# ToddThomson/Mila

Hardware: AMD Instinct MI355X
Metric: Gemma-4 12B decode tok/s (B=1, context 2048), 1xMI355X (higher is better)
Workload: dtype bf16; 1 GPU; Gemma-4 12B, weight policy bf16, B=1, prefill T=2048 then decode at positions 2048..; decode_mode=graph, replicas=1, parallelism=replicas only (no collective), bounded_local_kv=0

## Files before the change

### mila_amd/csrc/attention.hip

```cpp
#include "common.h"
#include "rms_common.h"
#include "rope_common.h"
#include "internal.h"
#include "attention_generic.h"
#include "attention_tiles.h"
#include "attention_decode_mfma.h"
#include "attention_decode_plan.h"

namespace mila {

__global__ __launch_bounds__(256) void kv_write_bf16_kernel(uint16_t* __restrict__ Kc, uint16_t* __restrict__ Vc,
                                                            const uint16_t* __restrict__ k,
                                                            const uint16_t* __restrict__ v, int64_t total_vec,
                                                            int chunk, int NKV, int HS, int start_pos, int capacity)
{
    const int hv = HS / 8;
    const int64_t stride = (int64_t)gridDim.x * 256;
    for (int64_t i = (int64_t)blockIdx.x * 256 + threadIdx.x; i < total_vec; i += stride)
    {
        const int e = (int)(i % hv);
        int64_t r = i / hv;
        const int n = (int)(r % NKV);
        r /= NKV;
        const int t = (int)(r % chunk);
        const int b = (int)(r / chunk);
        const int row = (start_pos + t) % capacity;
        const size_t dst = ((((size_t)b * NKV + n) * capacity + row) * hv + e) * 8;
        st16(Kc + dst, ld16(k + i * 8));
        st16(Vc + dst, ld16(v + i * 8));
    }
}

struct AttnParams
{
    uint16_t* Y;
    const uint16_t* Q;
    int64_t q_b_stride;
    uint16_t* K;
    uint16_t* V;
    float* scratch;
    int no_combine;
    const uint8_t* warm_a; int64_t warm_a_lines; int warm_a_blocks;
    const uint8_t* warm_b; int64_t warm_b_lines; int warm_b_blocks; int64_t warm_b_pair;
    uint32_t* tickets;
    int NH, NKV, capacity, position, window, splits;
    float scale;
    const int32_t* pos_dev;
    int flat;
    int64_t raw_b_stride;
    const uint16_t* q_raw;
    const uint16_t* k_raw;
    const uint16_t* v_raw;
    const uint16_t* qw;
    const uint16_t* kw;
    const uint16_t* vw;
    const float* cos_cache;
    const float* sin_cache;
    float eps;
};

template <int EPL>
__device__ __forceinline__ void load_row(uint32_t (&dst)[EPL / 2], const uint16_t* p)
{
    if constexpr (EPL == 8)
    {
        const u32x4 v = ld16(p);
        dst[0] = v[0]; dst[1] = v[1]; dst[2] = v[2]; dst[3] = v[3];
    }
    else if constexpr (EPL == 4)
    {
        const u32x2 v = *reinterpret_cast<const u32x2*>(p);
        dst[0] = v[0]; dst[1] = v[1];
    }
    else
    {
        dst[0] = *reinterpret_cast<const uint32_t*>(p);
    }
}

constexpr int kDecodeWaves = 8;

template <int HS>
__device__ __forceinline__ void head_row_post(const uint16_t* __restrict__ src, const uint16_t* __restrict__ w, bool rotate,
                                              const float* cos_row, const float* sin_row, float eps,
                                              uint16_t* dst_lds, uint16_t* dst_glb)
{
    constexpr int hv = HS / 16;
    const int lane = threadIdx.x & 63;
    const bool act = lane < hv;
    const int l2 = act ? lane : 0;
    const u32x4 xlo = ld16(src + (size_t)l2 * 8), xhi = ld16(src + (size_t)(l2 + hv) * 8);
    u32x4 wlo = u32x4{0u, 0u, 0u, 0u}, whi = wlo;
    if (w) { wlo = ld16(w + (size_t)l2 * 8); whi = ld16(w + (size_t)(l2 + hv) * 8); }
    const float rstd = rms_rstd_wave(src, HS, eps);
    if (act)
    {
        u32x4 lo, hi;
        if (w) { lo = rms_apply8(xlo, wlo, rstd, 0.0f); hi = rms_apply8(xhi, whi, rstd, 0.0f); }
        else { lo = rms_apply8_now(xlo, rstd); hi = rms_apply8_now(xhi, rstd); }
        if (rotate) rope_rotate8_vals(lo, hi, cos_row, sin_row, lane * 8);
        if (dst_lds) { st16(dst_lds + (size_t)lane * 8, lo); st16(dst_lds + (size_t)(lane + hv) * 8, hi); }
        if (dst_glb) { st16(dst_glb + (size_t)lane * 8, lo); st16(dst_glb + (size_t)(lane + hv) * 8, hi); }
    }
}

template <bool SC1>
__device__ __forceinline__ float partial_ld(const float* p)
{
    if constexpr (SC1)
        return __hip_atomic_load((const __attribute__((address_space(1))) float*)p, __ATOMIC_RELAXED, __HIP_MEMORY_SCOPE_AGENT);
    else
        return *p;
}
template <bool SC1>
__device__ __forceinline__ uint16_t combine_dim(const float* __restrict__ base, int HS, int splits, int d)
{
    const int STR = HS + 4;
    const int s = threadIdx.x & 63;
    float vals[16];
#pragma unroll
    for (int u = 0; u < 16; ++u) vals[u] = (u < splits) ? partial_ld<SC1>(base + (size_t)u * STR + d) : 0.0f;
    const float ms = (s < splits) ? partial_ld<SC1>(base + (size_t)s * STR + HS) : -INFINITY;
    const float ls = (s < splits) ? partial_ld<SC1>(base + (size_t)s * STR + HS + 1) : 0.0f;
    float acc = 0.0f;
    const float M = wave_max(ms);
    const float fs = (ms == -INFINITY) ? 0.0f : __expf(ms - M);
    const float L = wave_sum(ls * fs);
    const int n8 = (splits + 7) & ~7;
    for (int i0 = 0; i0 < n8; i0 += 16)
    {
        if (i0 > 0)
        {
#pragma unroll
            for (int u = 0; u < 16; ++u) vals[u] = (i0 + u < splits) ? partial_ld<SC1>(base + (size_t)(i0 + u) * STR + d) : 0.0f;
        }
#pragma unroll
        for (int u = 0; u < 16; ++u)
        {
            const float f = __uint_as_float(__builtin_amdgcn_readlane(__float_as_uint(fs), min(i0 + u, 63)));
            if (i0 + u < n8) acc = fmaf(vals[u], f, acc);
        }
    }
    return f32_to_bf16_bits(L > 0.0f ? acc / L : 0.0f);
}
__device__ __forceinline__ void partial_st_sc1(float* p, float v)
{
    __hip_atomic_store((__attribute__((address_space(1))) float*)p, v, __ATOMIC_RELAXED, __HIP_MEMORY_SCOPE_AGENT);
}

__device__ __forceinline__ void warm_lines(const uint8_t* __restrict__ base, int64_t nlines, int64_t tid, int64_t nthreads, float* never,
                                           int64_t pair = 0)
{
    uint32_t acc = 0;
    int64_t i = tid;
    auto at = [&](int64_t l) { return pair ? base + (l & 1) * pair + (l >> 1) * 128 : base + l * 128; };
    for (; i + 7 * nthreads < nlines; i += 8 * nthreads)
    {
        uint32_t v[8];
#pragma unroll
        for (int u = 0; u < 8; ++u) v[u] = *reinterpret_cast<const uint32_t*>(at(i + u * nthreads));
#pragma unroll
        for (int u = 0; u < 8; ++u) acc ^= v[u];
    }
    for (; i < nlines; i += nthreads) acc ^= *reinterpret_cast<const uint32_t*>(at(i));
    if (acc == 0x12345679u && never != nullptr) never[0] = 1.0f;
}

template <int HS, int GH, bool FUSED>
__global__ __launch_bounds__(kDecodeWaves * 64) void attn_decode_kernel(const AttnParams p)
{
    constexpr int NW = kDecodeWaves;
    constexpr int EPL = (HS >= 128) ? HS / 64 : 2;
    constexpr int NPAIR = EPL / 2;
    constexpr int ACTIVE = HS / EPL;
    constexpr int STR = HS + 2;
    extern __shared__ __attribute__((aligned(16))) unsigned char smem_raw[];
    float* sm = reinterpret_cast<float*>(smem_raw);
    uint16_t* qs = reinterpret_cast<uint16_t*>(smem_raw + (size_t)NW * GH * STR * sizeof(float));

    const int lane = threadIdx.x & 63, wave = threadIdx.x >> 6;
    const bool owner = lane < ACTIVE;
    const int GS = p.NH / p.NKV, hgroups = GS / GH;
    if (!p.flat && (int)blockIdx.x >= p.splits)
    {
        const int64_t wb = ((int64_t)(blockIdx.x - p.splits) * gridDim.y + blockIdx.y) * gridDim.z + blockIdx.z;
        warm_lines(p.warm_a, p.warm_a_lines, wb * (NW * 64) + threadIdx.x, (int64_t)p.warm_a_blocks * gridDim.y * gridDim.z * (NW * 64),
                   p.scratch);
        return;
    }
    const int ngrp = p.NKV * hgroups;
    const int split = p.flat ? (int)blockIdx.x / ngrp : (int)blockIdx.x, grp = p.flat ? (int)blockIdx.x % ngrp : (int)blockIdx.y;
    const int kvh = grp / hgroups, hg = grp % hgroups;
    const int h0 = kvh * GS + hg * GH;
    const int b = blockIdx.z;
    const int pos = p.pos_dev ? *p.pos_dev : p.position;
    const int len = pos + 1;
    const int band_begin = (p.window > 0) ? max(0, len - p.window) : 0;
    const int band = len - band_begin;
    const int chunk = (band + p.splits - 1) / p.splits;
    const int begin = band_begin + split * chunk;
    const int end = min(begin + chunk, len);
    const bool owns_new = FUSED && pos >= begin && pos < end;

    uint16_t* kbase = p.K + ((size_t)b * p.NKV + kvh) * p.capacity * HS;
    uint16_t* vbase = p.V + ((size_t)b * p.NKV + kvh) * p.capacity * HS;

    constexpr int PG = (HS >= 512) ? 4 : 8;
    struct KVG { uint32_t k[PG][NPAIR], v[PG][NPAIR]; };
    auto load_group = [&](KVG& gbuf, int base) {
#pragma unroll
        for (int j = 0; j < PG; ++j)
        {
            const int pp = base + NW * j;
            if (owner && pp < end && !(FUSED && pp == pos))
            {
                const size_t r = (size_t)(pp % p.capacity) * HS + lane * EPL;
                load_row<EPL>(gbuf.k[j], kbase + r);
                load_row<EPL>(gbuf.v[j], vbase + r);
            }
            else
            {
#pragma unroll
                for (int e = 0; e < NPAIR; ++e) { gbuf.k[j][e] = 0u; gbuf.v[j][e] = 0u; }
            }
        }
    };

    int base = begin + wave;
    KVG ga, gb;
    if (base < end) load_group(ga, base);

    uint32_t q[GH][NPAIR];
    if constexpr (FUSED)
    {
        const int half = HS / 2;
        const float* cos_row = p.cos_cache + (size_t)pos * half;
        const float* sin_row = p.sin_cache + (size_t)pos * half;
        const int nrows = GH + (owns_new ? 2 : 0);
        for (int r = wave; r < nrows; r += NW)
        {
            if (r < GH)
                head_row_post<HS>(p.q_raw + (size_t)b * p.raw_b_stride + (size_t)(h0 + r) * HS, p.qw, true, cos_row, sin_row, p.eps, qs + (size_t)r * HS, nullptr);
            else if (r == GH)
                head_row_post<HS>(p.k_raw + (size_t)b * p.raw_b_stride + (size_t)kvh * HS, p.kw, true, cos_row, sin_row, p.eps, qs + (size_t)GH * HS,
                                  (hg == 0) ? kbase + (size_t)(pos % p.capacity) * HS : nullptr);
            else
                head_row_post<HS>(p.v_raw + (size_t)b * p.raw_b_stride + (size_t)kvh * HS, p.vw, false, cos_row, sin_row, p.eps, qs + (size_t)(GH + 1) * HS,
                                  (hg == 0) ? vbase + (size_t)(pos % p.capacity) * HS : nullptr);
        }
        __syncthreads();
#pragma unroll
        for (int g = 0; g < GH; ++g)
        {
            if (owner) load_row<EPL>(q[g], qs + (size_t)g * HS + lane * EPL);
            else
            {
#pragma unroll
                for (int e = 0; e < NPAIR; ++e) q[g][e] = 0u;
            }
        }
    }
    else
    {
#pragma unroll
        for (int g = 0; g < GH; ++g)
        {
            const uint16_t* qp = p.Q + (size_t)b * (p.q_b_stride ? (size_t)p.q_b_stride : (size_t)p.NH * HS) + (size_t)(h0 + g) * HS + lane * EPL;
            if (owner) load_row<EPL>(q[g], qp);
            else
            {
#pragma unroll
                for (int e = 0; e < NPAIR; ++e) q[g][e] = 0u;
            }
        }
    }

    float m[GH], l[GH], o[GH][EPL];
#pragma unroll
    for (int g = 0; g < GH; ++g)
    {
        m[g] = -INFINITY;
        l[g] = 0.0f;
#pragma unroll
        for (int e = 0; e < EPL; ++e) o[g][e] = 0.0f;
    }

    auto patch_new = [&](KVG& gbuf, int base_) {
        if constexpr (FUSED)
        {
            if (owns_new)
            {
#pragma unroll
                for (int j = 0; j < PG; ++j)
                    if (base_ + NW * j == pos && owner)
                    {
                        load_row<EPL>(gbuf.k[j], qs + (size_t)GH * HS + lane * EPL);
                        load_row<EPL>(gbuf.v[j], qs + (size_t)(GH + 1) * HS + lane * EPL);
                    }
            }
        }
    };
    auto compute_group = [&](const KVG& gbuf, int base_) {
        float sc[PG][GH];
#pragma unroll
        for (int j = 0; j < PG; ++j)
#pragma unroll
            for (int g = 0; g < GH; ++g)
            {
                float a = 0.0f;
#pragma unroll
                for (int e = 0; e < NPAIR; ++e) a = dot2_bf16(as_bf16x2(q[g][e]), as_bf16x2(gbuf.k[j][e]), a);
                sc[j][g] = a;
            }
#pragma unroll
        for (int j = 0; j < PG; ++j)
#pragma unroll
            for (int g = 0; g < GH; ++g) sc[j][g] = wave_sum(sc[j][g]);
#pragma unroll
        for (int g = 0; g < GH; ++g)
        {
            float a[PG], mt = -INFINITY;
#pragma unroll
            for (int j = 0; j < PG; ++j)
            {
                a[j] = (base_ + NW * j < end) ? sc[j][g] * p.scale : -INFINITY;
                mt = fmaxf(mt, a[j]);
            }
            const float mn = fmaxf(m[g], mt);
            const float msafe = (mn == -INFINITY) ? 0.0f : mn;
            const float alpha = __expf(m[g] - msafe);
            float ex[PG], rs = 0.0f;
#pragma unroll
            for (int j = 0; j < PG; ++j) { ex[j] = __expf(a[j] - msafe); rs += ex[j]; }
            l[g] = l[g] * alpha + rs;
            m[g] = mn;
#pragma unroll
            for (int e = 0; e < NPAIR; ++e)
            {
                float lo = o[g][2 * e] * alpha, hi = o[g][2 * e + 1] * alpha;
#pragma unroll
                for (int j = 0; j < PG; ++j)
                {
                    lo = fmaf(ex[j], bf16_lo(gbuf.v[j][e]), lo);
                    hi = fmaf(ex[j], bf16_hi(gbuf.v[j][e]), hi);
                }
                o[g][2 * e] = lo;
                o[g][2 * e + 1] = hi;
            }
        }
    };
    for (;;)
    {
        if (base >= end) break;
        int nb = base + NW * PG;
        if (nb < end) load_group(gb, nb);
        patch_new(ga, base);
        compute_group(ga, base);
        base = nb;
        if (base >= end) break;
        nb = base + NW * PG;
        if (nb < end) load_group(ga, nb);
        patch_new(gb, base);
        compute_group(gb, base);
        base = nb;
    }

#pragma unroll
    for (int g = 0; g < GH; ++g)
    {
        float* dst = sm + ((size_t)wave * GH + g) * STR;
        if (owner)
        {
#pragma unroll
            for (int e = 0; e < EPL; ++e) dst[lane * EPL + e] = o[g][e];
        }
        if (lane == 0) { dst[HS] = m[g]; dst[HS + 1] = l[g]; }
    }
    __syncthreads();
    if (wave < GH)
    {
        const int g = wave;
        float M = -INFINITY;
#pragma unroll
        for (int w = 0; w < NW; ++w) M = fmaxf(M, sm[((size_t)w * GH + g) * STR + HS]);
        float L = 0.0f, acc[EPL];
#pragma unroll
        for (int e = 0; e < EPL; ++e) acc[e] = 0.0f;
#pragma unroll
        for (int w = 0; w < NW; ++w)
        {
            const float* src = sm + ((size_t)w * GH + g) * STR;
            const float mw = src[HS];
            const float f = (mw == -INFINITY) ? 0.0f : __expf(mw - M);
            L += src[HS + 1] * f;
            if (owner)
            {
#pragma unroll
                for (int e = 0; e < EPL; ++e) acc[e] += src[lane * EPL + e] * f;
            }
        }
        const int h = h0 + g;
        if (p.splits == 1)
        {
            const float inv = (L > 0.0f) ? 1.0f / L : 0.0f;
            uint16_t* y = p.Y + ((size_t)b * p.NH + h) * HS + lane * EPL;
            if (owner)
            {
#pragma unroll
                for (int e = 0; e < EPL; e += 2)
                    *reinterpret_cast<uint32_t*>(y + e) = pack_bf16x2(acc[e] * inv, acc[e + 1] * inv);
            }
        }
        else if (p.tickets == nullptr)
        {
            float* dst = p.scratch + (((size_t)b * p.NH + h) * p.splits + split) * (HS + 4);
            if (owner)
            {
#pragma unroll
                for (int e = 0; e < EPL; ++e) dst[lane * EPL + e] = acc[e];
            }
            if (lane == 0) { dst[HS] = M; dst[HS + 1] = L; }
        }
        else
        {
            float* dst = p.scratch + (((size_t)b * p.NH + h) * p.splits + split) * (HS + 4);
            if (owner)
            {
#pragma unroll
                for (int e = 0; e < EPL; ++e) partial_st_sc1(dst + lane * EPL + e, acc[e]);
            }
            if (lane == 0) { partial_st_sc1(dst + HS, M); partial_st_sc1(dst + HS + 1, L); }
            asm volatile("s_waitcnt vmcnt(0)" ::: "memory");
        }
    }
    if (p.splits > 1 && p.tickets != nullptr)
    {
        __shared__ int s_last;
        __syncthreads();
        uint32_t* tk = p.tickets + (size_t)b * gridDim.y + blockIdx.y;
        if (threadIdx.x == 0)
        {
            const uint32_t t = __hip_atomic_fetch_add(tk, 1u, __ATOMIC_ACQ_REL, __HIP_MEMORY_SCOPE_AGENT);
            const int last = (t == (uint32_t)(p.splits - 1));
            if (last) __hip_atomic_store(tk, 0u, __ATOMIC_RELAXED, __HIP_MEMORY_SCOPE_AGENT);
            s_last = last;
        }
        __syncthreads();
        if (s_last)
        {
            for (int idx = threadIdx.x; idx < GH * HS; idx += NW * 64)
            {
                const int g = idx / HS, d = idx % HS;
                const int h = h0 + g;
                const float* base = p.scratch + ((size_t)b * p.NH + h) * p.splits * (HS + 4);
                p.Y[((size_t)b * p.NH + h) * HS + d] = combine_dim<true>(base, HS, p.splits, d);
            }
        }
    }
}

__global__ __launch_bounds__(64) void attn_combine_kernel(uint16_t* __restrict__ Y, const float* __restrict__ scratch, int NH,
                                                          int HS, int splits, const uint8_t* __restrict__ warm, int64_t warm_lines_n, int64_t warm_pair, int flat_gh)
{
    int h = blockIdx.x, zc = blockIdx.z;
    const int b = blockIdx.y;
    if (flat_gh > 0)
    {
        const int ngroups = NH / flat_gh, grp = (int)blockIdx.x % ngroups, r = (int)blockIdx.x / ngroups;
        h = grp * flat_gh + r % flat_gh;
        zc = r / flat_gh;
    }
    else if ((int)blockIdx.z >= HS / 64)
    {
        const int64_t wb = ((int64_t)(blockIdx.z - HS / 64) * gridDim.y + blockIdx.y) * gridDim.x + blockIdx.x;
        warm_lines(warm, warm_lines_n, wb * 64 + threadIdx.x, (int64_t)(gridDim.z - HS / 64) * gridDim.y * gridDim.x * 64, nullptr, warm_pair);
        return;
    }
    const int d = zc * 64 + threadIdx.x;
    const float* base = scratch + ((size_t)b * NH + h) * splits * (HS + 4);
    Y[((size_t)b * NH + h) * HS + d] = combine_dim<false>(base, HS, splits, d);
}


template <int HS>
__global__ __launch_bounds__(256) void attn_decode_mfma_kernel(const AttnParams p)
{
    extern __shared__ __attribute__((aligned(16))) unsigned char smem_mfma[];
    const int pos = p.pos_dev ? *p.pos_dev : p.position;
    const MfmaDecodeArgs a{p.Q, p.q_b_stride, p.scratch, p.NH, p.NKV, p.capacity, pos + 1, p.window, p.splits, p.scale};
    attn_decode_mfma_body<HS>(a, MfmaStageBf16<HS>{p.K, p.V}, smem_mfma);
}

__global__ __launch_bounds__(256) void attn_combine_many_kernel(uint16_t* __restrict__ Y, const float* __restrict__ scratch, int NH, int HS, int splits)
{
    __shared__ float s_acc[4][64], s_m[4], s_l[4];
    const int h = blockIdx.x, b = blockIdx.y, lane = threadIdx.x & 63, wave = threadIdx.x >> 6;
    const int d = blockIdx.z * 64 + lane;
    const int STR = HS + 4;
    const int s0 = wave * 64, n = min(64, splits - s0);
    const float* base = scratch + (((size_t)b * NH + h) * splits + s0) * STR;
    float acc = 0.0f, M = -INFINITY, L = 0.0f;
    if (n > 0)
    {
        float vals[16];
#pragma unroll
        for (int u = 0; u < 16; ++u) vals[u] = (u < n) ? base[(size_t)u * STR + d] : 0.0f;
        const float ms = (lane < n) ? base[(size_t)lane * STR + HS] : -INFINITY;
        const float ls = (lane < n) ? base[(size_t)lane * STR + HS + 1] : 0.0f;
        M = wave_max(ms);
        const float fs = (ms == -INFINITY) ? 0.0f : __expf(ms - M);
        L = wave_sum(ls * fs);
        const int n16 = (n + 15) & ~15;
        for (int i0 = 0; i0 < n16; i0 += 16)
        {
            if (i0 > 0)
            {
#pragma unroll
                for (int u = 0; u < 16; ++u) vals[u] = (i0 + u < n) ? base[(size_t)(i0 + u) * STR + d] : 0.0f;
            }
#pragma unroll
            for (int u = 0; u < 16; ++u)
            {
                const float f = __uint_as_float(__builtin_amdgcn_readlane(__float_as_uint(fs), min(i0 + u, 63)));
                acc = fmaf(vals[u], f, acc);
            }
        }
    }
    s_acc[wave][lane] = acc;
    if (lane == 0) { s_m[wave] = M; s_l[wave] = L; }
    __syncthreads();
    if (wave == 0)
    {
        float Mt = fmaxf(fmaxf(s_m[0], s_m[1]), fmaxf(s_m[2], s_m[3]));
        float Lt = 0.0f, out = 0.0f;
#pragma unroll
        for (int w = 0; w < 4; ++w)
        {
            const float f = (s_m[w] == -INFINITY) ? 0.0f : __expf(s_m[w] - Mt);
            Lt = fmaf(s_l[w], f, Lt);
            out = fmaf(s_acc[w][lane], f, out);
        }
        Y[((size_t)b * NH + h) * HS + d] = f32_to_bf16_bits(Lt > 0.0f ? out / Lt : 0.0f);
    }
}

enum DecodeForm { DF_SCALAR, DF_MFMA, DF_GENERIC };
struct DecodePlan
{
    DecodeForm form;
    int splits, band_max;
    int gh, hgroups;
    int flat;
    bool prologue;
    size_t partial_floats;
    size_t scratch_need;
};

constexpr int kMaxSplits = 64;
constexpr int kMaxSplitsMfma = 256;
static int g_tune_positions_per_split = 64;
MILA_TUNE("attn.positions_per_split", g_tune_positions_per_split);
static int g_attn_max_wgs = 256;
MILA_TUNE("attn.max_workgroups", g_attn_max_wgs);
static int g_attn_gh512 = 2;
MILA_TUNE("attn.heads_per_group_512", g_attn_gh512);
static int g_tune_decode_mfma = 1;
MILA_TUNE("attn.mfma_decode", g_tune_decode_mfma);
static int g_tune_kvfp8_mfma = 1;
MILA_TUNE("attn.kvfp8_mfma_decode", g_tune_kvfp8_mfma);
static int g_mfma_min_band = 8192;
MILA_TUNE("attn.mfma_min_band", g_mfma_min_band);
static int g_attn_xcd_local = 0;
MILA_TUNE("attn.xcd_local", g_attn_xcd_local);

static int band_bucket(int len, int capacity)
{
    int b = 4096;
    while (b < len && b < capacity) b <<= 1;
    return min(b, capacity);
}
static int heads_per_group(int GS, int HS) { return HS >= 512 ? (GS >= g_attn_gh512 && g_attn_gh512 == 4 ? 4 : (GS >= 2 ? 2 : 1)) : (GS >= 4 ? 4 : GS); }
static int decode_splits(int B, int NKV, int hgroups, int band)
{
    const int cap = max(1, g_attn_max_wgs / (NKV * hgroups * B));
    const int pps = g_tune_positions_per_split >= 8 ? g_tune_positions_per_split : 64;
    return max(1, min(min((band + pps - 1) / pps, cap), kMaxSplits));
}
static bool mfma_decode_applies(int NH, int NKV, int HS, int band_max)
{
    return g_tune_decode_mfma && HS == 512 && NKV > 0 && (NH / NKV) % 16 == 0 && band_max >= g_mfma_min_band;
}
static int mfma_decode_splits(int B, int NH, int NKV, int band_max)
{
    const int groups = NKV * ((NH / NKV) / 16) * B;
    const int s = (band_max + 127) / 128;
    return max(1, min(min(s, max(1, kNumCU / groups)), kMaxSplitsMfma));
}
static size_t decode_scratch_bytes(int B, int NH, int HS, int splits, bool q_rows)
{
    return (size_t)B * NH * splits * (HS + 4) * sizeof(float) + (q_rows ? (size_t)B * NH * HS * 2 : 0);
}

static DecodePlan plan_decode(int B, int NH, int NKV, int HS, int capacity, int window, int len_hint, bool fused, bool hooks, bool kvfp8 = false)
{
    const bool scalar_only = kvfp8 && !g_tune_kvfp8_mfma;
    DecodePlan d{};
    const int GS = NH / NKV;
    const bool split_kernel = HS == 64 || HS == 128 || HS == 256 || HS == 512;
    d.band_max = (window > 0 && window < capacity) ? window : (len_hint > 0 ? band_bucket(len_hint, capacity) : capacity);
    d.gh = heads_per_group(GS, HS);
    d.hgroups = GS / d.gh;
    if (mfma_decode_applies(NH, NKV, HS, d.band_max) && !hooks && !scalar_only)
    {
        d.form = DF_MFMA;
        d.splits = mfma_decode_splits(B, NH, NKV, d.band_max);
        d.prologue = fused;
    }
    else
    {
        d.form = split_kernel ? DF_SCALAR : DF_GENERIC;
        d.splits = decode_splits(B, NKV, d.hgroups, d.band_max);
        d.flat = (g_attn_xcd_local && split_kernel && (NKV * d.hgroups) % 8 == 0 && !hooks) ? 1 : 0;
    }
    d.partial_floats = (size_t)B * NH * d.splits * (HS + 4);
    d.scratch_need = (d.form == DF_MFMA || (d.form == DF_SCALAR && d.splits > 1)) ? decode_scratch_bytes(B, NH, HS, d.splits, d.prologue) : 0;
    return d;
}
int launch_attn_combine_many(uint16_t* Y, const float* partials, int B, int NH, int HS, int splits, hipStream_t s)
{
    hipLaunchKernelGGL(attn_combine_many_kernel, dim3(NH, B, HS / 64), dim3(256), 0, s, Y, partials, NH, HS, splits);
    return check_hip(hipGetLastError(), "attn_combine_many");
}
static int launch_decode_mfma(const AttnParams& p, int B, hipStream_t s)
{
    constexpr int HS = 512;
    note_form("attn_decode_mfma");
    static bool attr_set = false;
    const size_t lds = mfma_decode_lds_bytes<HS>();
    if (!attr_set)
    {
        int rc = check_hip(hipFuncSetAttribute(reinterpret_cast<const void*>(attn_decode_mfma_kernel<HS>), hipFuncAttributeMaxDynamicSharedMemorySize, (int)lds), "hipFuncSetAttribute(attn_decode_mfma)");
        if (rc) return rc;
        attr_set = true;
    }
    const int n16 = (p.NH / p.NKV) / 16;
    hipLaunchKernelGGL((attn_decode_mfma_kernel<HS>), dim3(p.splits, p.NKV * n16, B), dim3(256), lds, s, p);
    int rc = check_hip(hipGetLastError(), "attn_decode_mfma");
    if (rc) return rc;
    return launch_attn_combine_many(p.Y, p.scratch, B, p.NH, HS, p.splits, s);
}

template <int HS, int GH, bool FUSED>
static int launch_decode(const AttnParams& p, int B, hipStream_t s)
{
    const int hgroups = (p.NH / p.NKV) / GH;
    note_form("attn_decode");
    const size_t lds = (size_t)kDecodeWaves * GH * (HS + 2) * sizeof(float) + (size_t)(GH + 2) * HS * 2;
    const int wa = (p.warm_a && p.warm_a_lines > 0) ? p.warm_a_blocks : 0;
    if (p.flat)
    {
        hipLaunchKernelGGL((attn_decode_kernel<HS, GH, FUSED>), dim3(p.NKV * hgroups * p.splits, 1, B), dim3(kDecodeWaves * 64), lds, s, p);
        int rc = check_hip(hipGetLastError(), "attn_decode (xcd-local)");
        if (rc || p.splits <= 1) return rc;
        hipLaunchKernelGGL(attn_combine_kernel, dim3(p.NH * (HS / 64), B, 1), dim3(64), 0, s, p.Y, p.scratch, p.NH, HS, p.splits, nullptr, 0, 0, GH);
        return check_hip(hipGetLastError(), "attn_combine (xcd-local)");
    }
    hipLaunchKernelGGL((attn_decode_kernel<HS, GH, FUSED>), dim3(p.splits + wa, p.NKV * hgroups, B), dim3(kDecodeWaves * 64), lds, s, p);
    int rc = check_hip(hipGetLastError(), "attn_decode");
    if (rc) return rc;
    if (p.splits > 1 && !p.no_combine && !p.tickets)
    {
        const int wbk = (p.warm_b && p.warm_b_lines > 0) ? p.warm_b_blocks : 0;
        hipLaunchKernelGGL(attn_combine_kernel, dim3(p.NH, B, HS / 64 + wbk), dim3(64), 0, s, p.Y, p.scratch, p.NH, HS, p.splits, p.warm_b,
                           p.warm_b_lines, p.warm_b_pair, 0);
        rc = check_hip(hipGetLastError(), "attn_combine");
    }
    return rc;
}

template <int HS, bool FUSED>
static int dispatch_gs(const AttnParams& p, int B, hipStream_t s)
{
    const int GS = p.NH / p.NKV;
    if (GS != 1 && GS != 2 && GS != 4 && GS != 8 && GS != 16 && GS != 32)
        return set_error(MILA_E_UNSUPPORTED, "attention: group size %d (NH/NKV) must be 1,2,4,8,16 or 32", GS);
    switch (heads_per_group(GS, HS))
    {
        case 1: return launch_decode<HS, 1, FUSED>(p, B, s);
        case 2: return launch_decode<HS, 2, FUSED>(p, B, s);
        default: return launch_decode<HS, 4, FUSED>(p, B, s);
    }
}

template <bool FUSED>
static int dispatch_hs(int HS, const AttnParams& p, int B, hipStream_t s)
{
    switch (HS)
    {
        case 64: return dispatch_gs<64, FUSED>(p, B, s);
        case 128: return dispatch_gs<128, FUSED>(p, B, s);
        case 256: return dispatch_gs<256, FUSED>(p, B, s);
        case 512: return dispatch_gs<512, FUSED>(p, B, s);
        default:
            if constexpr (!FUSED)
            {
                if (p.pos_dev) return set_error(MILA_E_UNSUPPORTED, "attention: the device-position form needs a head size of 64, 128, 256 or 512 (got %d)", HS);
                const int64_t qbs = p.q_b_stride ? p.q_b_stride : (int64_t)p.NH * HS;
                GenericAttnParams g{p.Y, p.Q, p.K, p.V, qbs, qbs, (int64_t)p.NKV * p.capacity * HS, (int64_t)p.capacity * HS, HS,
                                    B, 1, p.NH, p.NKV, HS, p.capacity, p.position, p.window, p.scale};
                return launch_attn_generic(g, s);
            }
            return set_error(MILA_E_UNSUPPORTED, "attention: head size %d must be 64, 128, 256 or 512", HS);
    }
}

static int run_decode(const DecodePlan& d, AttnParams p, int B, int HS, size_t scratch_bytes, const char* who, hipStream_t stream)
{
    const bool fused = p.q_raw != nullptr;
    p.splits = d.splits;
    p.flat = d.flat;
    if (d.scratch_need && (!p.scratch || scratch_bytes < d.scratch_need))
        return set_error(MILA_E_SCRATCH_TOO_SMALL, "%s: scratch %zu bytes < required %zu", who, scratch_bytes, d.scratch_need);
    if (d.form != DF_MFMA) return fused ? dispatch_hs<true>(HS, p, B, stream) : dispatch_hs<false>(HS, p, B, stream);
    if (d.prologue)
    {
        uint16_t* q_tmp = reinterpret_cast<uint16_t*>(p.scratch + d.partial_floats);
        for (int b = 0; b < B; ++b)
        {
            uint16_t* kc = p.K + (size_t)b * p.NKV * p.capacity * HS;
            uint16_t* vc = p.V + (size_t)b * p.NKV * p.capacity * HS;
            const size_t ro = (size_t)b * p.raw_b_stride;
            const int rc = p.pos_dev ? mila_cdna4_fused_qkv_post_devpos(q_tmp + (size_t)b * p.NH * HS, kc, vc, p.q_raw + ro, p.k_raw + ro, p.v_raw + ro, p.qw, p.kw, p.vw, p.cos_cache,
                                                                        p.sin_cache, p.NH, p.NKV, HS, p.pos_dev, p.capacity, p.eps, reinterpret_cast<mila_stream_t>(stream))
                                     : mila_cdna4_fused_qkv_post(q_tmp + (size_t)b * p.NH * HS, kc, vc, p.q_raw + ro, p.k_raw + ro, p.v_raw + ro, p.qw, p.kw, p.vw, p.cos_cache,
                                                                 p.sin_cache, p.NH, p.NKV, HS, p.position, p.capacity, p.eps, reinterpret_cast<mila_stream_t>(stream));
            if (rc) return rc;
        }
        p.Q = q_tmp;
        p.q_b_stride = 0;
    }
    return launch_decode_mfma(p, B, stream);
}

static int unfused_decode(const char* who, uint16_t* Y, const uint16_t* Q, int64_t q_b_stride, const uint16_t* Kc, const uint16_t* Vc, void* scratch, size_t scratch_bytes, int B,
                          int NH, int NKV, int HS, int capacity, int position, const int32_t* pos_dev, int len_hint, int window, float scale, hipStream_t stream)
{
    AttnParams p{};
    p.Y = Y; p.Q = Q; p.q_b_stride = q_b_stride; p.K = const_cast<uint16_t*>(Kc); p.V = const_cast<uint16_t*>(Vc); p.scratch = reinterpret_cast<float*>(scratch);
    p.NH = NH; p.NKV = NKV; p.capacity = capacity; p.position = position; p.pos_dev = pos_dev; p.window = window; p.scale = scale;
    return run_decode(plan_decode(B, NH, NKV, HS, capacity, window, len_hint, false, false), p, B, HS, scratch_bytes, who, stream);
}

enum { FD_BATCH = 1, FD_TICKETS = 2, FD_PARTIALS = 4 };
static int fused_decode(const char* who, const mila_fused_attn_args& a, int B, int64_t raw_b_stride, int flags, hipStream_t stream)
{
    MILA_REQUIRE((a.Y || (flags & FD_PARTIALS)) && a.Kc && a.Vc && a.q_raw && a.k_raw && a.v_raw && a.qw && a.kw && a.cos_cache && a.sin_cache &&
                 (a.tickets || !(flags & FD_TICKETS)), "%s: null pointer", who);
    if (flags & FD_BATCH)
    {
        MILA_REQUIRE(B > 0 && a.NH > 0 && a.NKV > 0 && a.NH % a.NKV == 0, "%s: bad sizes (B=%d NH=%d NKV=%d)", who, B, a.NH, a.NKV);
        MILA_REQUIRE(B == 1 || raw_b_stride >= (int64_t)a.NKV * a.HS, "%s: raw_b_stride %lld is shorter than a K row", who, (long long)raw_b_stride);
    }
    else
        MILA_REQUIRE(a.NH > 0 && a.NKV > 0 && a.NH % a.NKV == 0, "%s: bad head counts (NH=%d NKV=%d)", who, a.NH, a.NKV);
    MILA_REQUIRE(a.capacity > 0 && a.window >= 0 && (a.position_dev || a.position >= 0), "%s: bad sizes", who);
    MILA_REQUIRE(a.HS % 16 == 0, "%s: HS=%d must be a multiple of 16", who, a.HS);
    MILA_REQUIRE(a.warm_a_blocks >= 0 && a.warm_a_blocks <= 64 && a.warm_b_blocks >= 0 && a.warm_b_blocks <= 64, "%s: warm block counts must be in [0, 64]", who);
    if (a.tickets)
        MILA_REQUIRE(a.ticket_count >= mila_cdna4_attn_decode_ticket_count(1, a.NH), "%s: %zu tickets < required %zu", who, a.ticket_count,
                     mila_cdna4_attn_decode_ticket_count(1, a.NH));
    AttnParams p{};
    p.Y = a.Y; p.K = a.Kc; p.V = a.Vc; p.scratch = reinterpret_cast<float*>(a.scratch);
    p.NH = a.NH; p.NKV = a.NKV; p.capacity = a.capacity; p.position = a.position; p.pos_dev = a.position_dev; p.window = a.window; p.scale = a.scale;
    p.q_raw = a.q_raw; p.k_raw = a.k_raw; p.v_raw = a.v_raw; p.raw_b_stride = raw_b_stride; p.qw = a.qw; p.kw = a.kw; p.vw = a.vw;
    p.cos_cache = a.cos_cache; p.sin_cache = a.sin_cache; p.eps = a.eps;
    p.tickets = a.tickets;
    p.no_combine = (flags & FD_PARTIALS) ? 1 : 0;
    if (a.warm_a && a.warm_a_bytes >= 128 && a.warm_a_blocks > 0) { p.warm_a = (const uint8_t*)a.warm_a; p.warm_a_lines = (int64_t)(a.warm_a_bytes / 128); p.warm_a_blocks = a.warm_a_blocks; }
    if (a.warm_b && a.warm_b_bytes >= 128 && a.warm_b_blocks > 0) { p.warm_b = (const uint8_t*)a.warm_b; p.warm_b_lines = (int64_t)(a.warm_b_bytes / 128); p.warm_b_blocks = a.warm_b_blocks; p.warm_b_pair = (int64_t)a.warm_b_pair_offset; }
    const DecodePlan d = plan_decode(B, a.NH, a.NKV, a.HS, a.capacity, a.window, a.position_dev ? a.position : a.position + 1, true,
                                     p.tickets || p.no_combine || p.warm_a || p.warm_b);
    if (flags & FD_PARTIALS) MILA_REQUIRE(d.splits > 1, "%s: this (window, capacity) runs unsplit; use fused_attn_decode_bf16", who);
    if (!a.position_dev)
    {
        const int len = a.position + 1, band = (a.window > 0 && a.window < len) ? a.window : len;
        MILA_REQUIRE(band <= a.capacity, "%s: live band %d exceeds the cache capacity %d", who, band, a.capacity);
    }
    return run_decode(d, p, B, a.HS, a.scratch_bytes, who, stream);
}
static mila_fused_attn_args fused_args(uint16_t* Y, uint16_t* Kc, uint16_t* Vc, const uint16_t* q_raw, const uint16_t* k_raw, const uint16_t* v_raw, const uint16_t* qw,
                                       const uint16_t* kw, const uint16_t* vw, const float* cos_cache, const float* sin_cache, void* scratch, size_t scratch_bytes,
                                       uint32_t* tickets, size_t ticket_count, int NH, int NKV, int HS, int capacity, int position, const int32_t* position_dev, int window,
                                       float scale, float eps)
{
    return mila_fused_attn_args{Y, Kc, Vc, q_raw, k_raw, v_raw, qw, kw, vw, cos_cache, sin_cache, scratch, scratch_bytes, tickets, ticket_count, nullptr, 0, 0, nullptr, 0, 0, 0,
                                NH, NKV, HS, capacity, position, position_dev, window, scale, eps};
}

KvFp8DecodeShape plan_decode_kvfp8(int B, int NH, int NKV, int HS, int capacity, int window, int len_hint)
{
    const DecodePlan d = plan_decode(B, NH, NKV, HS, capacity, window, len_hint, false, false, true);
    return KvFp8DecodeShape{d.form == DF_MFMA, d.splits, d.gh, d.hgroups, d.scratch_need};
}
int launch_attn_combine(uint16_t* Y, const float* partials, int B, int NH, int HS, int splits, hipStream_t s)
{
    hipLaunchKernelGGL(attn_combine_kernel, dim3(NH, B, HS / 64), dim3(64), 0, s, Y, partials, NH, HS, splits, nullptr, 0, 0, 0);
    return check_hip(hipGetLastError(), "attn_combine");
}
// ... 206 lines not shown
```

### mila_amd/csrc/rms_common.h

```cpp
#pragma once
#include "common.h"

namespace mila {

__device__ __forceinline__ float sumsq8(const u32x4 v, float acc)
{
#pragma unroll
    for (int d = 0; d < 4; ++d)
    {
        const float lo = bf16_lo(v[d]), hi = bf16_hi(v[d]);
        acc = fmaf(lo, lo, acc);
        acc = fmaf(hi, hi, acc);
    }
    return acc;
}

template <int NW>
__device__ __forceinline__ float rms_rstd_block(const uint16_t* __restrict__ x, int dim, float eps, float* red)
{
    const int lane = threadIdx.x & 63, wib = threadIdx.x >> 6;
    const int nx16 = dim / 8, G = (nx16 + 63) / 64;
    for (int g = wib; g < G; g += NW)
    {
        const int c = 64 * g + lane;
        float s = c < nx16 ? sumsq8(ld16(x + (size_t)c * 8), 0.0f) : 0.0f;
        s = wave_sum(s);
        if (lane == 0) red[g] = s;
    }
    __syncthreads();
    float t = 0.0f;
    for (int g = 0; g < G; ++g) t += red[g];
    return rsqrtf(t / (float)dim + eps);
}
__device__ __forceinline__ float rms_rstd_wave(const uint16_t* __restrict__ x, int dim, float eps)
{
    const int lane = threadIdx.x & 63;
    float ss = 0.0f;
    for (int i = lane; i < dim / 8; i += 64) ss = sumsq8(ld16(x + (size_t)i * 8), ss);
    ss = wave_sum(ss);
    return rsqrtf(ss / (float)dim + eps);
}

__device__ __forceinline__ float rms_apply1(float x, float w, float rstd, float w_offset, float b)
{
    return x * rstd * (w + w_offset) + b;
}
__device__ __forceinline__ u32x4 rms_apply8(const u32x4 x, const u32x4 w, float rstd, float w_offset)
{
    u32x4 y;
#pragma unroll
    for (int d = 0; d < 4; ++d)
        y[d] = pack_bf16x2(rms_apply1(bf16_lo(x[d]), bf16_lo(w[d]), rstd, w_offset, 0.0f),
                           rms_apply1(bf16_hi(x[d]), bf16_hi(w[d]), rstd, w_offset, 0.0f));
    return y;
}
__device__ __forceinline__ u32x4 rms_apply8_bias(const u32x4 x, const u32x4 w, const u32x4 b, float rstd, float w_offset)
{
    u32x4 y;
#pragma unroll
    for (int d = 0; d < 4; ++d)
        y[d] = pack_bf16x2(rms_apply1(bf16_lo(x[d]), bf16_lo(w[d]), rstd, w_offset, bf16_lo(b[d])),
                           rms_apply1(bf16_hi(x[d]), bf16_hi(w[d]), rstd, w_offset, bf16_hi(b[d])));
    return y;
}
__device__ __forceinline__ u32x4 sandwich_tail8(const u32x4 a, const u32x4 rr, float post_scale)
{
    u32x4 r;
#pragma unroll
    for (int d = 0; d < 4; ++d)
    {
        float lo = round_bf16(bf16_lo(rr[d]) + bf16_lo(a[d]));
        float hi = round_bf16(bf16_hi(rr[d]) + bf16_hi(a[d]));
        if (post_scale != 1.0f) { lo = lo * post_scale; hi = hi * post_scale; }
        r[d] = pack_bf16x2(lo, hi);
    }
    return r;
}

__device__ __forceinline__ u32x4 rms_apply8_now(const u32x4 x, float rstd)
{
    u32x4 y;
#pragma unroll
    for (int d = 0; d < 4; ++d)
        y[d] = pack_bf16x2(rms_apply1(bf16_lo(x[d]), 1.0f, rstd, 0.0f, 0.0f), rms_apply1(bf16_hi(x[d]), 1.0f, rstd, 0.0f, 0.0f));
    return y;
}

}
```

Measured before the change: 221.9 tok/s.

## Restructure decode attention prologue to issue loads early and remove divides

Splits the fused q/k/v RMS-norm plus RoPE head-row preprocessing into a request phase and a finish phase. All global loads (rows, weights, cos/sin, first KV group) are issued before any reduction or sync, so their latencies overlap. KV ring indexing switches from per-row modulo to incremental wrap with precomputed steps, head-group math uses host-precomputed shifts and masks, and loads become unconditional with clamped addresses and masking applied afterwards. This removes serialized load latency and integer divides at the cost of extra register pressure and redundant loads for inactive rows. The head-group shift assumes a power-of-two group count, and rms_rstd_wave_request only covers dim up to 512.

```diff
diff --git a/mila_amd/csrc/attention.hip b/mila_amd/csrc/attention.hip
--- a/mila_amd/csrc/attention.hip
+++ b/mila_amd/csrc/attention.hip
@@ -57,6 +57,7 @@
     const float* cos_cache;
     const float* sin_cache;
     float eps;
+    int gs, hgroups, hg_shift, ngrp, ring_step, ring_gstep;
 };
 
 template <int EPL>
@@ -80,25 +81,33 @@
 
 constexpr int kDecodeWaves = 8;
 
+struct HeadRowReq { u32x4 xlo, xhi, wlo, whi, xs; };
 template <int HS>
-__device__ __forceinline__ void head_row_post(const uint16_t* __restrict__ src, const uint16_t* __restrict__ w, bool rotate,
-                                              const float* cos_row, const float* sin_row, float eps,
-                                              uint16_t* dst_lds, uint16_t* dst_glb)
+__device__ __forceinline__ HeadRowReq head_row_request(const uint16_t* __restrict__ src, const uint16_t* __restrict__ w)
 {
     constexpr int hv = HS / 16;
     const int lane = threadIdx.x & 63;
-    const bool act = lane < hv;
-    const int l2 = act ? lane : 0;
-    const u32x4 xlo = ld16(src + (size_t)l2 * 8), xhi = ld16(src + (size_t)(l2 + hv) * 8);
-    u32x4 wlo = u32x4{0u, 0u, 0u, 0u}, whi = wlo;
-    if (w) { wlo = ld16(w + (size_t)l2 * 8); whi = ld16(w + (size_t)(l2 + hv) * 8); }
-    const float rstd = rms_rstd_wave(src, HS, eps);
-    if (act)
+    const int l2 = lane < hv ? lane : 0;
+    const uint16_t* wp = w ? w : src;
+    HeadRowReq r;
+    r.xs = rms_rstd_wave_request(src, HS);
+    r.xlo = ld16(src + (size_t)l2 * 8); r.xhi = ld16(src + (size_t)(l2 + hv) * 8);
+    r.wlo = ld16(wp + (size_t)l2 * 8); r.whi = ld16(wp + (size_t)(l2 + hv) * 8);
+    return r;
+}
+template <int HS>
+__device__ __forceinline__ void head_row_finish(const HeadRowReq& r, bool has_w, bool rotate, f32x4 c0, f32x4 c1, f32x4 s0, f32x4 s1, float eps,
+                                                uint16_t* dst_lds, uint16_t* dst_glb)
+{
+    constexpr int hv = HS / 16;
+    const int lane = threadIdx.x & 63;
+    const float rstd = rms_rstd_wave_finish(r.xs, HS, eps);
+    if (lane < hv)
     {
         u32x4 lo, hi;
-        if (w) { lo = rms_apply8(xlo, wlo, rstd, 0.0f); hi = rms_apply8(xhi, whi, rstd, 0.0f); }
-        else { lo = rms_apply8_now(xlo, rstd); hi = rms_apply8_now(xhi, rstd); }
-        if (rotate) rope_rotate8_vals(lo, hi, cos_row, sin_row, lane * 8);
+        if (has_w) { lo = rms_apply8(r.xlo, r.wlo, rstd, 0.0f); hi = rms_apply8(r.xhi, r.whi, rstd, 0.0f); }
+        else { lo = rms_apply8_now(r.xlo, rstd); hi = rms_apply8_now(r.xhi, rstd); }
+        if (rotate) rope_rotate8_regs(lo, hi, c0, c1, s0, s1);
         if (dst_lds) { st16(dst_lds + (size_t)lane * 8, lo); st16(dst_lds + (size_t)(lane + hv) * 8, hi); }
         if (dst_glb) { st16(dst_glb + (size_t)lane * 8, lo); st16(dst_glb + (size_t)(lane + hv) * 8, hi); }
     }
@@ -117,11 +126,16 @@
 {
     const int STR = HS + 4;
     const int s = threadIdx.x & 63;
+    const int last = splits - 1;
     float vals[16];
 #pragma unroll
-    for (int u = 0; u < 16; ++u) vals[u] = (u < splits) ? partial_ld<SC1>(base + (size_t)u * STR + d) : 0.0f;
-    const float ms = (s < splits) ? partial_ld<SC1>(base + (size_t)s * STR + HS) : -INFINITY;
-    const float ls = (s < splits) ? partial_ld<SC1>(base + (size_t)s * STR + HS + 1) : 0.0f;
+    for (int u = 0; u < 16; ++u) vals[u] = partial_ld<SC1>(base + (size_t)min(u, last) * STR + d);
+    float ms = partial_ld<SC1>(base + (size_t)min(s, last) * STR + HS);
+    float ls = partial_ld<SC1>(base + (size_t)min(s, last) * STR + HS + 1);
+#pragma unroll
+    for (int u = 0; u < 16; ++u) vals[u] = (u < splits) ? vals[u] : 0.0f;
+    ms = (s < splits) ? ms : -INFINITY;
+    ls = (s < splits) ? ls : 0.0f;
     float acc = 0.0f;
     const float M = wave_max(ms);
     const float fs = (ms == -INFINITY) ? 0.0f : __expf(ms - M);
@@ -132,7 +146,9 @@
         if (i0 > 0)
         {
 #pragma unroll
-            for (int u = 0; u < 16; ++u) vals[u] = (i0 + u < splits) ? partial_ld<SC1>(base + (size_t)(i0 + u) * STR + d) : 0.0f;
+            for (int u = 0; u < 16; ++u) vals[u] = partial_ld<SC1>(base + (size_t)min(i0 + u, last) * STR + d);
+#pragma unroll
+            for (int u = 0; u < 16; ++u) vals[u] = (i0 + u < splits) ? vals[u] : 0.0f;
         }
 #pragma unroll
         for (int u = 0; u < 16; ++u)
@@ -178,9 +194,9 @@
     float* sm = reinterpret_cast<float*>(smem_raw);
     uint16_t* qs = reinterpret_cast<uint16_t*>(smem_raw + (size_t)NW * GH * STR * sizeof(float));
 
-    const int lane = threadIdx.x & 63, wave = threadIdx.x >> 6;
+    const int lane = threadIdx.x & 63, wave = __builtin_amdgcn_readfirstlane(threadIdx.x >> 6);
     const bool owner = lane < ACTIVE;
-    const int GS = p.NH / p.NKV, hgroups = GS / GH;
+    const unsigned lane_off = (unsigned)(owner ? lane : 0) * EPL;
     if (!p.flat && (int)blockIdx.x >= p.splits)
     {
         const int64_t wb = ((int64_t)(blockIdx.x - p.splits) * gridDim.y + blockIdx.y) * gridDim.z + blockIdx.z;
@@ -188,91 +204,116 @@
                    p.scratch);
         return;
     }
-    const int ngrp = p.NKV * hgroups;
-    const int split = p.flat ? (int)blockIdx.x / ngrp : (int)blockIdx.x, grp = p.flat ? (int)blockIdx.x % ngrp : (int)blockIdx.y;
-    const int kvh = grp / hgroups, hg = grp % hgroups;
-    const int h0 = kvh * GS + hg * GH;
+    const int split = p.flat ? (int)blockIdx.x / p.ngrp : (int)blockIdx.x, grp = p.flat ? (int)blockIdx.x % p.ngrp : (int)blockIdx.y;
+    const int kvh = grp >> p.hg_shift, hg = grp & (p.hgroups - 1);
+    const int h0 = kvh * p.gs + hg * GH;
     const int b = blockIdx.z;
     const int pos = p.pos_dev ? *p.pos_dev : p.position;
+
+    uint16_t* kbase = p.K + ((size_t)b * p.NKV + kvh) * p.capacity * HS;
+    uint16_t* vbase = p.V + ((size_t)b * p.NKV + kvh) * p.capacity * HS;
+    asm volatile("" ::"s"(kbase), "s"(vbase));
+
+    uint32_t q[GH][NPAIR];
+    HeadRowReq req;
+    bool has_w = false;
+    const uint16_t *idle_k, *idle_v;
+    if constexpr (FUSED)
+    {
+        const size_t rb = (size_t)b * p.raw_b_stride;
+        idle_k = p.k_raw + rb + (size_t)kvh * HS;
+        idle_v = p.v_raw + rb + (size_t)kvh * HS;
+        if (wave < GH + 2)
+        {
+            const uint16_t* src = (wave < GH) ? p.q_raw + rb + (size_t)(h0 + wave) * HS : (wave == GH ? idle_k : idle_v);
+            const uint16_t* w = (wave < GH) ? p.qw : (wave == GH ? p.kw : p.vw);
+            has_w = w != nullptr;
+            req = head_row_request<HS>(src, w);
+        }
+    }
+    else
+    {
+        const uint16_t* qrow = p.Q + (size_t)b * (p.q_b_stride ? (size_t)p.q_b_stride : (size_t)p.NH * HS) + (size_t)h0 * HS;
+        idle_k = idle_v = qrow;
+#pragma unroll
+        for (int g = 0; g < GH; ++g) load_row<EPL>(q[g], qrow + (size_t)g * HS + lane_off);
+        __builtin_amdgcn_sched_barrier(0);
+    }
+
     const int len = pos + 1;
     const int band_begin = (p.window > 0) ? max(0, len - p.window) : 0;
     const int band = len - band_begin;
-    const int chunk = (band + p.splits - 1) / p.splits;
+    const int chunk = (int)((unsigned)(band + p.splits - 1) / (unsigned)p.splits);
     const int begin = band_begin + split * chunk;
     const int end = min(begin + chunk, len);
     const bool owns_new = FUSED && pos >= begin && pos < end;
-
-    uint16_t* kbase = p.K + ((size_t)b * p.NKV + kvh) * p.capacity * HS;
-    uint16_t* vbase = p.V + ((size_t)b * p.NKV + kvh) * p.capacity * HS;
+    const int endc = FUSED ? min(end, pos) : end;
+
+    f32x4 c0 = f32x4{0.0f, 0.0f, 0.0f, 0.0f}, c1 = c0, s0 = c0, s1 = c0;
+    if constexpr (FUSED)
+    {
+        if (wave <= GH)
+        {
+            constexpr int half = HS / 2;
+            const unsigned co = (unsigned)(lane < HS / 16 ? lane : 0) * 8;
+            const float* cos_row = p.cos_cache + (size_t)pos * half;
+            const float* sin_row = p.sin_cache + (size_t)pos * half;
+            c0 = *reinterpret_cast<const f32x4*>(cos_row + co); c1 = *reinterpret_cast<const f32x4*>(cos_row + co + 4);
+            s0 = *reinterpret_cast<const f32x4*>(sin_row + co); s1 = *reinterpret_cast<const f32x4*>(sin_row + co + 4);
+        }
+    }
 
     constexpr int PG = (HS >= 512) ? 4 : 8;
     struct KVG { uint32_t k[PG][NPAIR], v[PG][NPAIR]; };
-    auto load_group = [&](KVG& gbuf, int base) {
+    auto load_group = [&](KVG& gbuf, int base_, unsigned row_) {
+        const bool any = base_ < endc;
+        const uint16_t* kb = any ? kbase : idle_k;
+        const uint16_t* vb = any ? vbase : idle_v;
+        unsigned r = any ? row_ : 0u;
 #pragma unroll
         for (int j = 0; j < PG; ++j)
         {
-            const int pp = base + NW * j;
-            if (owner && pp < end && !(FUSED && pp == pos))
-            {
-                const size_t r = (size_t)(pp % p.capacity) * HS + lane * EPL;
-                load_row<EPL>(gbuf.k[j], kbase + r);
-                load_row<EPL>(gbuf.v[j], vbase + r);
-            }
-            else
-            {
-#pragma unroll
-                for (int e = 0; e < NPAIR; ++e) { gbuf.k[j][e] = 0u; gbuf.v[j][e] = 0u; }
-            }
+            if (j > 0 && base_ + NW * j < endc)
+            {
+                r += (unsigned)p.ring_step;
+                if (r >= (unsigned)p.capacity) r -= (unsigned)p.capacity;
+            }
+            load_row<EPL>(gbuf.k[j], kb + (size_t)r * HS + lane_off);
+            load_row<EPL>(gbuf.v[j], vb + (size_t)r * HS + lane_off);
+        }
+#pragma unroll
+        for (int j = 0; j < PG; ++j)
+        {
+            const bool keep = owner && base_ + NW * j < endc;
+#pragma unroll
+            for (int e = 0; e < NPAIR; ++e) { gbuf.k[j][e] = keep ? gbuf.k[j][e] : 0u; gbuf.v[j][e] = keep ? gbuf.v[j][e] : 0u; }
         }
     };
 
     int base = begin + wave;
+    unsigned row = (unsigned)base % (unsigned)p.capacity;
     KVG ga, gb;
-    if (base < end) load_group(ga, base);
-
-    uint32_t q[GH][NPAIR];
+    load_group(ga, base, row);
+
     if constexpr (FUSED)
     {
-        const int half = HS / 2;
-        const float* cos_row = p.cos_cache + (size_t)pos * half;
-        const float* sin_row = p.sin_cache + (size_t)pos * half;
         const int nrows = GH + (owns_new ? 2 : 0);
-        for (int r = wave; r < nrows; r += NW)
-        {
-            if (r < GH)
-                head_row_post<HS>(p.q_raw + (size_t)b * p.raw_b_stride + (size_t)(h0 + r) * HS, p.qw, true, cos_row, sin_row, p.eps, qs + (size_t)r * HS, nullptr);
-            else if (r == GH)
-                head_row_post<HS>(p.k_raw + (size_t)b * p.raw_b_stride + (size_t)kvh * HS, p.kw, true, cos_row, sin_row, p.eps, qs + (size_t)GH * HS,
-                                  (hg == 0) ? kbase + (size_t)(pos % p.capacity) * HS : nullptr);
-            else
-                head_row_post<HS>(p.v_raw + (size_t)b * p.raw_b_stride + (size_t)kvh * HS, p.vw, false, cos_row, sin_row, p.eps, qs + (size_t)(GH + 1) * HS,
-                                  (hg == 0) ? vbase + (size_t)(pos % p.capacity) * HS : nullptr);
+        if (wave < nrows)
+        {
+            uint16_t* glb = nullptr;
+            if (wave >= GH && hg == 0) glb = (wave == GH ? kbase : vbase) + (size_t)(pos % p.capacity) * HS;
+            head_row_finish<HS>(req, has_w, wave <= GH, c0, c1, s0, s1, p.eps, qs + (size_t)wave * HS, glb);
         }
         __syncthreads();
 #pragma unroll
+        for (int g = 0; g < GH; ++g) load_row<EPL>(q[g], qs + (size_t)g * HS + lane_off);
+    }
+    if (!owner)
+    {
+#pragma unroll
         for (int g = 0; g < GH; ++g)
-        {
-            if (owner) load_row<EPL>(q[g], qs + (size_t)g * HS + lane * EPL);
-            else
-            {
-#pragma unroll
-                for (int e = 0; e < NPAIR; ++e) q[g][e] = 0u;
-            }
-        }
-    }
-    else
-    {
-#pragma unroll
-        for (int g = 0; g < GH; ++g)
-        {
-            const uint16_t* qp = p.Q + (size_t)b * (p.q_b_stride ? (size_t)p.q_b_stride : (size_t)p.NH * HS) + (size_t)(h0 + g) * HS + lane * EPL;
-            if (owner) load_row<EPL>(q[g], qp);
-            else
-            {
-#pragma unroll
-                for (int e = 0; e < NPAIR; ++e) q[g][e] = 0u;
-            }
-        }
+#pragma unroll
+            for (int e = 0; e < NPAIR; ++e) q[g][e] = 0u;
     }
 
     float m[GH], l[GH], o[GH][EPL];
@@ -349,17 +390,23 @@
             }
         }
     };
+    auto next_row = [&](unsigned r) {
+        r += (unsigned)p.ring_gstep;
+        return r >= (unsigned)p.capacity ? r - (unsigned)p.capacity : r;
+    };
     for (;;)
     {
         if (base >= end) break;
         int nb = base + NW * PG;
-        if (nb < end) load_group(gb, nb);
+        row = next_row(row);
+        if (nb < end) load_group(gb, nb, row);
         patch_new(ga, base);
         compute_group(ga, base);
         base = nb;
         if (base >= end) break;
         nb = base + NW * PG;
-        if (nb < end) load_group(ga, nb);
+        row = next_row(row);
+        if (nb < end) load_group(ga, nb, row);
         patch_new(gb, base);
         compute_group(gb, base);
         base = nb;
@@ -651,9 +698,13 @@
 }
 
 template <int HS, int GH, bool FUSED>
-static int launch_decode(const AttnParams& p, int B, hipStream_t s)
-{
+static int launch_decode(const AttnParams& p_in, int B, hipStream_t s)
+{
+    AttnParams p = p_in;
     const int hgroups = (p.NH / p.NKV) / GH;
+    p.gs = p.NH / p.NKV; p.hgroups = hgroups; p.hg_shift = __builtin_ctz((unsigned)hgroups); p.ngrp = p.NKV * hgroups;
+    p.ring_step = kDecodeWaves % p.capacity;
+    p.ring_gstep = (kDecodeWaves * (HS >= 512 ? 4 : 8)) % p.capacity;
     note_form("attn_decode");
     const size_t lds = (size_t)kDecodeWaves * GH * (HS + 2) * sizeof(float) + (size_t)(GH + 2) * HS * 2;
     const int wa = (p.warm_a && p.warm_a_lines > 0) ? p.warm_a_blocks : 0;
diff --git a/mila_amd/csrc/rms_common.h b/mila_amd/csrc/rms_common.h
--- a/mila_amd/csrc/rms_common.h
+++ b/mila_amd/csrc/rms_common.h
@@ -37,6 +37,18 @@
     const int lane = threadIdx.x & 63;
     float ss = 0.0f;
     for (int i = lane; i < dim / 8; i += 64) ss = sumsq8(ld16(x + (size_t)i * 8), ss);
+    ss = wave_sum(ss);
+    return rsqrtf(ss / (float)dim + eps);
+}
+__device__ __forceinline__ u32x4 rms_rstd_wave_request(const uint16_t* __restrict__ x, int dim)
+{
+    const int lane = threadIdx.x & 63;
+    return ld16(x + (size_t)min(lane, dim / 8 - 1) * 8);
+}
+__device__ __forceinline__ float rms_rstd_wave_finish(const u32x4 chunk, int dim, float eps)
+{
+    const int lane = threadIdx.x & 63;
+    float ss = (lane < dim / 8) ? sumsq8(chunk, 0.0f) : 0.0f;
     ss = wave_sum(ss);
     return rsqrtf(ss / (float)dim + eps);
 }
```

Result: no change. 223.7 tok/s (median of 5 runs) (+0.8%).
